# reczoo/RecBox

Hardware: AMD Instinct MI355X
Metric: samples/sec fwd+bwd, Criteo-shaped batch 65 536; embedding HBM GB/s vs roofline (higher is better)
Workload: dtype f32; 1 GPU; FM (recbox.ranking) Criteo-shaped 26 sparse + 13 dense, dim 16, batch 65536 per GPU, uniform ids (8 distinct batches resident in HBM, replayed in rotation), fused path, hipGraph replay (one captured step per resident batch), dense-grad autograd contract (persistent grad buffer, rows of the previous step re-zeroed), no optimiser step; global_batch=65536, batch_per_gpu=65536, parallelism=dp1

## Files before the change

### recbox_amd/csrc/rbx_bwd_common.h

```cpp
#pragma once
#include "rbx_internal.h"

namespace rbx {

constexpr int kSortThreads = 256;
#define RBX_SORT_ITEMS 8
constexpr int kSortItems = RBX_SORT_ITEMS;
constexpr int kSortTile = kSortThreads * kSortItems;
constexpr int kChainTiles = 64;
constexpr int kChainPasses = 4;
constexpr int kRadix = 256;
#define RBX_MAX_RADIX_BITS 8
constexpr int kMaxRadixBits = RBX_MAX_RADIX_BITS;
#define RBX_CHUNK 40
constexpr int kChunk = RBX_CHUNK;
constexpr unsigned kLocalBits = 26;
constexpr unsigned kLocalMask = (1u << kLocalBits) - 1u;
constexpr int kNumSamples = 256;

struct KeyField {
  const void* ids;
  long long stride_b;
  int stride_l;
  int vocab;
  int mask_id;
  int pad_id;
  unsigned row_base;
  unsigned lk_off;
  short seq_len;
  unsigned char dtype, pool;
  int reserved;
};
struct KeyPack { KeyField f[RBX_MAX_FIELDS]; };
// ... 2 lines not shown
  float* grad;
  float* grad2;
  const float* table;
  unsigned row_base;
  int out_off;
  short dim;
  short seq_len;
  unsigned char pool, slot;
  short reserved;
  int table_stride;
  int reserved2;
};
struct RedPack { RedField f[RBX_MAX_FIELDS]; };

struct SegPack {
  unsigned tile0[RBX_MAX_FIELDS + 1];
  unsigned lk0[RBX_MAX_FIELDS + 1];
  unsigned row0[RBX_MAX_FIELDS];
  unsigned char first_pass[RBX_MAX_FIELDS];
  int n;
};
static_assert(sizeof(KeyPack) + sizeof(SegPack) + 96 <= 4096, "build_keys_kernel's arguments must fit the 4 KiB kernarg segment");

__device__ __forceinline__ void seg_of_tile(const SegPack& S, unsigned tile, int* seg, unsigned* first, unsigned* count) {
  int lo = 0, hi = S.n - 1;
  while (lo < hi) {
    const int mid = (lo + hi + 1) >> 1;
    if (S.tile0[mid] <= tile) lo = mid; else hi = mid - 1;
  }
  *seg = lo;
  const unsigned f = S.lk0[lo] + (tile - S.tile0[lo]) * static_cast<unsigned>(kSortTile);
  const unsigned end = S.lk0[lo + 1];
  *first = f;
  *count = (end - f < static_cast<unsigned>(kSortTile)) ? end - f : static_cast<unsigned>(kSortTile);
}

template <int RB>
__device__ __forceinline__ unsigned seg_digit(unsigned key, unsigned sentinel, unsigned row0, int shift) {
  const unsigned local = (key == sentinel) ? 0xFFFFFFFFu : key - row0;
  return (local >> shift) & ((1u << RB) - 1u);
}

struct NumField {
  const void* ids;
  float* grad;
  long long stride_b;
  int out_off;
  short dim;
  unsigned char dtype, reserved;
};
struct NumPack { NumField f[RBX_MAX_FIELDS]; };

struct BwdPlan {
  int n_cat = 0, n_num = 0;
  KeyPack keys;
  RedPack red;
  NumPack num;
// ... 144 lines not shown
```

### recbox_amd/csrc/rbx_embed_bwd.hip

```cpp
#include <stdlib.h>
#include "rbx_segreduce.h"

namespace rbx {

static size_t align_up(size_t v, size_t a) { return (v + a - 1) / a * a; }

static int g_sort_chained = -1;
static bool sort_chained_on() {
  if (g_sort_chained < 0) {
    const char* e = getenv("RBX_SORT_CHAINED");
    g_sort_chained = (e != nullptr && e[0] == '0') ? 0 : 1;
  }
  return g_sort_chained != 0;
}

int make_plan(const rbx_field_t* fields, int n, int64_t B, const float* dout, int64_t stride_b, BwdPlan* p,
              int extra_dim, const unsigned long long* lookups_of) {
  if (fields == nullptr || n <= 0 || n > RBX_MAX_FIELDS) return fail(RBX_ERR_INVALID, "bad field array");
  FieldPack tmp;
  int rc = pack_fields(fields, n, B, true, &tmp);
  if (rc != RBX_OK) return rc;
  unsigned long long lookups = 0, rows = 0;
  const float* seen_table[RBX_MAX_FIELDS];
  unsigned seen_base[RBX_MAX_FIELDS];
// ... 79 lines not shown
    unsigned tiles = 0, lk = 0;
    unsigned long long max_rows = 1;
    unsigned long long rows_of_seg[RBX_MAX_FIELDS];
    int c = 0;
    while (c < p->n_cat) {
      int end = last_field_of_table[field_table[c]];
      unsigned long long seg_rows = 0;
      unsigned seg_lk = 0;
      const unsigned row0 = p->keys.f[c].row_base;
      int t_lo = field_table[c], t_hi = field_table[c];
      for (int k = c; k <= end; ++k) {
        if (last_field_of_table[field_table[k]] > end) end = last_field_of_table[field_table[k]];
        if (field_table[k] > t_hi) t_hi = field_table[k];
        if (field_table[k] < t_lo) t_lo = field_table[k];
        seg_lk += field_lookups[k];
      }
      for (int t = t_lo; t <= t_hi; ++t) seg_rows += static_cast<unsigned long long>(seen_vocab[t]);
      if (seg_lk > 0) {
        S.tile0[S.n] = tiles;
        S.lk0[S.n] = lk;
        S.row0[S.n] = row0;
        rows_of_seg[S.n] = seg_rows;
        ++S.n;
        tiles += (seg_lk + kSortTile - 1) / kSortTile;
        lk += seg_lk;
        if (seg_rows > max_rows) max_rows = seg_rows;
      }
      c = end + 1;
    }
    S.tile0[S.n] = tiles;
    S.lk0[S.n] = lk;
    p->n_tiles = tiles;
    unsigned max_nt = 0;
    for (int g = 0; g < S.n; ++g)
      if (S.tile0[g + 1] - S.tile0[g] > max_nt) max_nt = S.tile0[g + 1] - S.tile0[g];
    p->chained = max_nt <= static_cast<unsigned>(kChainTiles);
    int bits = 1;
    while ((1ull << bits) <= max_rows) ++bits;
    p->passes = (bits + kMaxRadixBits - 1) / kMaxRadixBits;
    const int per = (bits + p->passes - 1) / p->passes;
    p->radix_bits = per <= 8 ? 8 : (per <= 10 ? 10 : 11);
    for (int g = 0; g < S.n; ++g) {
      int sb = 1;
      while ((1ull << sb) <= rows_of_seg[g]) ++sb;
      const int need = (sb + p->radix_bits - 1) / p->radix_bits;
      S.first_pass[g] = static_cast<unsigned char>(p->passes - need);
    }
  }
  {
    int c = static_cast<int>(p->n_lookups / 32768u) / 8 * 8;
    if (c < 16) c = 16;
    if (c > kChunk) c = kChunk;
    p->chunk = c;
  }
  p->n_chunks = (p->n_lookups + p->chunk - 1) / p->chunk;
  p->num_blocks = static_cast<unsigned>((B + kNumSamples - 1) / kNumSamples);
  size_t o = 0;
  const size_t nl = align_up(static_cast<size_t>(p->n_lookups) * 4, 256);
  p->off_keys[0] = o; o += nl;
  p->off_keys[1] = o; o += nl;
  p->off_vals[0] = o; o += nl;
  p->off_vals[1] = o; o += nl;
  const size_t radix = static_cast<size_t>(1) << p->radix_bits;
  p->chained = sort_chained_on() && p->chained && p->passes <= kChainPasses && p->radix_bits == 8;
  p->off_hist = o;
  o += p->chained ? align_up((2 * static_cast<size_t>(p->n_tiles) * radix + p->n_tiles + static_cast<size_t>(p->segs.n) * radix) *
                             p->passes * 4, 256)
                  : align_up(static_cast<size_t>(p->n_tiles) * radix * 4 + 4, 256);
  p->off_ssum = o; o += align_up((static_cast<size_t>(p->n_tiles) * radix / 4096 + 2) * 4, 256);
  p->sum_stride = p->max_dim + extra_dim;
  p->off_head = o; o += align_up(static_cast<size_t>(p->n_chunks) * p->sum_stride * 4, 256);
  p->off_tail = o; o += align_up(static_cast<size_t>(p->n_chunks) * p->sum_stride * 4, 256);
  p->off_flags = o; o += align_up(static_cast<size_t>(p->n_chunks) * 4, 256);
  p->off_fin = o; o += align_up((2 * static_cast<size_t>(p->n_chunks) + 3 + kLongSlots) * 4, 256);
  p->off_long = o; o += align_up(static_cast<size_t>(kLongSlots) * p->sum_stride * 4, 256);
  p->off_num = o; o += align_up(static_cast<size_t>(p->n_num) * p->num_blocks * p->max_dim * 4, 256);
  p->bytes = o + 256;
  return RBX_OK;
}


template <int RB>
__global__ __launch_bounds__(kSortThreads) void build_keys_kernel(const KeyPack P, const int n_cat, const SegPack S,
                                                         const unsigned sentinel, unsigned* __restrict__ keys0,
                                                         unsigned* __restrict__ vals0, unsigned* __restrict__ keys1,
                                                         unsigned* __restrict__ vals1, int* __restrict__ status,
                                                         unsigned* __restrict__ fin, unsigned* __restrict__ hist,
                                                         const int chain_passes, const unsigned n_tiles) {
  constexpr int R = 1 << RB;
  constexpr int kCP = (RB == 8) ? kChainPasses : 1;
  if (blockIdx.x == 0 && threadIdx.x == 0) {
    fin[0] = 0;
    fin[1] = 0;
    fin[2] = 0;
  }
  __shared__ KeyField sf[RBX_MAX_FIELDS];
  {
    const int words = n_cat * static_cast<int>(sizeof(KeyField) / 4);
    const int* src = reinterpret_cast<const int*>(&P);
    int* dst = reinterpret_cast<int*>(sf);
    for (int i = threadIdx.x; i < words; i += blockDim.x) dst[i] = src[i];
  }
  __shared__ unsigned cnt[kCP][R];
  for (int d = threadIdx.x; d < kCP * R; d += kSortThreads) (&cnt[0][0])[d] = 0;
  __syncthreads();
  int seg;
  unsigned tile0, tile_n;
  seg_of_tile(S, blockIdx.x, &seg, &tile0, &tile_n);
  const unsigned row0 = S.row0[seg];
  const int fp = S.first_pass[seg];
  unsigned* __restrict__ keys = (fp & 1) ? keys1 : keys0;
  unsigned* __restrict__ vals = (fp & 1) ? vals1 : vals0;
#pragma unroll
  for (int it = 0; it < kSortItems; ++it) {
    const unsigned off = it * kSortThreads + threadIdx.x;
    if (off >= tile_n) break;
    const unsigned j = tile0 + off;
    int lo = 0, hi = n_cat - 1;
    while (lo < hi) {
      const int mid = (lo + hi + 1) >> 1;
      if (sf[mid].lk_off <= j) lo = mid; else hi = mid - 1;
    }
    const KeyField& fd = sf[lo];
    const unsigned local = j - fd.lk_off;
    const unsigned L = static_cast<unsigned>(fd.seq_len);
    const unsigned b = local / L;
    const unsigned l = local - b * L;
    const long long id = load_id(fd.ids, static_cast<long long>(b) * fd.stride_b + static_cast<long long>(l) * fd.stride_l,
                                 fd.dtype);
    unsigned key = sentinel;
    if (id < 0 || id >= fd.vocab) {
      if (status != nullptr) atomicOr(status, 1);
    } else {
      const bool id_pool = fd.pool == RBX_POOL_MEAN_ID || fd.pool == RBX_POOL_SUM_ID;
      if (id != fd.pad_id && !(id_pool && id == fd.mask_id)) key = fd.row_base + static_cast<unsigned>(id);
    }
    keys[j] = key;
    vals[j] = (static_cast<unsigned>(lo) << kLocalBits) | local;
    if (chain_passes > 0) {
#pragma unroll
      for (int k = 0; k < kCP; ++k)
        if (fp + k < chain_passes) atomicAdd(&cnt[k][seg_digit<RB>(key, sentinel, row0, k * RB)], 1u);
    } else if (fp == 0) {
      atomicAdd(&cnt[0][seg_digit<RB>(key, sentinel, row0, 0)], 1u);
    }
  }
  if (chain_passes > 0) {
    __syncthreads();
    const size_t plane = static_cast<size_t>(n_tiles) * R;
    unsigned* flags = hist + 2 * plane * chain_passes;
    for (int k = 0; fp + k < chain_passes; ++k) {
      unsigned* h = hist + plane * (fp + k) + static_cast<size_t>(blockIdx.x) * R;
      for (int d = threadIdx.x; d < R; d += kSortThreads) h[d] = cnt[k < kCP ? k : 0][d];
      if (threadIdx.x == 0) flags[static_cast<size_t>(fp + k) * n_tiles + blockIdx.x] = 0u;
    }
    return;
  }
  if (fp != 0) return;
  __syncthreads();
  const unsigned t_in = blockIdx.x - S.tile0[seg], nt = S.tile0[seg + 1] - S.tile0[seg];
  unsigned* h = hist + static_cast<size_t>(S.tile0[seg]) * R + t_in;
  for (int d = threadIdx.x; d < R; d += kSortThreads) h[static_cast<size_t>(d) * nt] = cnt[0][d];
}

template <int RB>
__global__ __launch_bounds__(kSortThreads) void radix_hist_kernel(const unsigned* __restrict__ keys, const SegPack S,
                                                                  const unsigned sentinel, const int pass,
                                                                  unsigned* __restrict__ hist) {
  constexpr int R = 1 << RB;
  __shared__ unsigned cnt[R];
  int seg;
  unsigned tile0, tile_n;
  seg_of_tile(S, blockIdx.x, &seg, &tile0, &tile_n);
  if (pass < S.first_pass[seg]) return;
  const int shift = (pass - S.first_pass[seg]) * RB;
  for (int d = threadIdx.x; d < R; d += kSortThreads) cnt[d] = 0;
  __syncthreads();
  const unsigned row0 = S.row0[seg];
#pragma unroll
  for (int i = 0; i < kSortItems; ++i) {
    const unsigned off = i * kSortThreads + threadIdx.x;
    if (off < tile_n) atomicAdd(&cnt[seg_digit<RB>(keys[tile0 + off], sentinel, row0, shift)], 1u);
  }
  __syncthreads();
  const unsigned t_in = blockIdx.x - S.tile0[seg], nt = S.tile0[seg + 1] - S.tile0[seg];
  unsigned* h = hist + static_cast<size_t>(S.tile0[seg]) * R + t_in;
  for (int d = threadIdx.x; d < R; d += kSortThreads) h[static_cast<size_t>(d) * nt] = cnt[d];
}

constexpr int kScanSlice = 4096;
constexpr int kMaxFusedSlices = 4 * kSortThreads;

__device__ __forceinline__ unsigned block_scan_1024x4(unsigned (&v)[4], unsigned* wave_tot, unsigned* total) {
  const int lane = threadIdx.x & 63, wid = threadIdx.x >> 6;
  const unsigned mine = v[0] + v[1] + v[2] + v[3];
  unsigned inc = mine;
#pragma unroll
  for (int o = 1; o < 64; o <<= 1) {
    const unsigned t = __shfl_up(inc, o, 64);
    if (lane >= o) inc += t;
  }
  if (lane == 63) wave_tot[wid] = inc;
  __syncthreads();
  unsigned wbase = 0, all = 0;
#pragma unroll
  for (int w = 0; w < 16; ++w) {
    const unsigned t = wave_tot[w];
    if (w < wid) wbase += t;
    all += t;
  }
  *total = all;
  return wbase + inc - mine;
}

// ... 14 lines not shown
  if (threadIdx.x == 0) slice_sum[blockIdx.x] = total;
}

__global__ __launch_bounds__(1024) void radix_scan_sums_kernel(unsigned* __restrict__ sums, const unsigned len) {
  __shared__ unsigned wave_tot[16];
  unsigned carry = 0;
  for (unsigned base = 0; base < len; base += kScanSlice) {
    const unsigned i0 = base + threadIdx.x * 4;
    unsigned v[4];
#pragma unroll
    for (int k = 0; k < 4; ++k) v[k] = (i0 + k < len) ? sums[i0 + k] : 0u;
    unsigned total;
    unsigned run = carry + block_scan_1024x4(v, wave_tot, &total);
#pragma unroll
    for (int k = 0; k < 4; ++k) {
      if (i0 + k < len) sums[i0 + k] = run;
      run += v[k];
    }
    carry += total;
    __syncthreads();
  }
}

template <int RB, bool CHAIN>
__global__ __launch_bounds__(kSortThreads) void radix_scatter_kernel(const unsigned* __restrict__ keys_in,
                                                                     const unsigned* __restrict__ vals_in,
                                                                     unsigned* __restrict__ keys_out,
                                                                     unsigned* __restrict__ vals_out, const SegPack S,
                                                                     const unsigned sentinel, const int pass,
                                                                     const unsigned* __restrict__ hist,
                                                                     const unsigned* __restrict__ slice_sum,
                                                                     const unsigned n_slices, const bool raw_sums,
                                                                     unsigned* __restrict__ chain, const int passes,
                                                                     const unsigned n_tiles) {
  constexpr int R = 1 << RB;
  constexpr int DPT = R / kSortThreads;
  constexpr int kWaves = kSortThreads / 64;
  constexpr int kPerWave = kSortTile / kWaves;
  constexpr int kSteps = kPerWave / 64;
  __shared__ unsigned wcnt[kWaves][R];
  __shared__ unsigned dstart[R];
  __shared__ unsigned gbase[R];
  __shared__ unsigned skey[kSortTile];
  __shared__ unsigned sval[kSortTile];
  const int lane = threadIdx.x & 63, wid = threadIdx.x >> 6;
  int seg;
  unsigned tile0, tile_n;
  seg_of_tile(S, blockIdx.x, &seg, &tile0, &tile_n);
  if (pass < S.first_pass[seg]) return;
  const int shift = (pass - S.first_pass[seg]) * RB;
  const unsigned row0 = S.row0[seg];
  const unsigned t_in = blockIdx.x - S.tile0[seg], nt = S.tile0[seg + 1] - S.tile0[seg];
  const size_t hfirst = static_cast<size_t>(S.tile0[seg]) * R;
  const size_t hbase = hfirst + t_in;
  const unsigned seg_lk0 = S.lk0[seg];
  for (int i = threadIdx.x; i < kWaves * R; i += kSortThreads) (&wcnt[0][0])[i] = 0;
  unsigned chain_excl[DPT], chain_before[DPT];
  const size_t plane = static_cast<size_t>(n_tiles) * R;
  const bool first_of_seg = pass == S.first_pass[seg];
  if constexpr (CHAIN) {
    __shared__ unsigned ctot[kWaves];
    const unsigned* T = chain + plane * pass + static_cast<size_t>(S.tile0[seg]) * R;
    unsigned* G = chain + (2 * plane + n_tiles) * passes;
    unsigned tot[DPT];
    unsigned mine = 0;
    if (first_of_seg) {
#pragma unroll
      for (int q = 0; q < DPT; ++q) {
        const int d = threadIdx.x * DPT + q;
        unsigned a = 0, b = 0;
#pragma unroll 8
        for (unsigned t = 0; t < nt; ++t) {
          const unsigned c = T[static_cast<size_t>(t) * R + d];
          a += c;
          b += (t < t_in) ? c : 0u;
        }
        tot[q] = a;
        chain_before[q] = b;
        mine += a;
      }
      if (t_in == 0) {
        for (int k = pass + 1; k < passes; ++k) {
          const unsigned* Tk = chain + plane * k + static_cast<size_t>(S.tile0[seg]) * R;
#pragma unroll
          for (int q = 0; q < DPT; ++q) {
            const int d = threadIdx.x * DPT + q;
            unsigned a = 0;
#pragma unroll 8
            for (unsigned t = 0; t < nt; ++t) a += Tk[static_cast<size_t>(t) * R + d];
            G[(static_cast<size_t>(k) * S.n + seg) * R + d] = a;
          }
        }
      }
    } else {
#pragma unroll
      for (int q = 0; q < DPT; ++q) {
        tot[q] = G[(static_cast<size_t>(pass) * S.n + seg) * R + threadIdx.x * DPT + q];
        chain_before[q] = 0;
        mine += tot[q];
      }
    }
    unsigned inc = mine;
#pragma unroll
    for (int o = 1; o < 64; o <<= 1) {
      const unsigned u = __shfl_up(inc, o, 64);
      if (lane >= o) inc += u;
    }
    if (lane == 63) ctot[wid] = inc;
    __syncthreads();
    unsigned run = inc - mine;
    for (int w = 0; w < wid; ++w) run += ctot[w];
#pragma unroll
    for (int q = 0; q < DPT; ++q) {
      chain_excl[q] = run;
      run += tot[q];
    }
  } else if (raw_sums) {
    __shared__ unsigned spre[kMaxFusedSlices];
    __shared__ unsigned stot[kWaves];
    const unsigned i0 = threadIdx.x * 4;
    unsigned t[4];
#pragma unroll
    for (int q = 0; q < 4; ++q) t[q] = (i0 + q < n_slices) ? slice_sum[i0 + q] : 0u;
    const unsigned mine = t[0] + t[1] + t[2] + t[3];
    unsigned inc = mine;
#pragma unroll
    for (int o = 1; o < 64; o <<= 1) {
      const unsigned u = __shfl_up(inc, o, 64);
      if (lane >= o) inc += u;
    }
    if (lane == 63) stot[wid] = inc;
    __syncthreads();
    unsigned run = inc - mine;
    for (int w = 0; w < wid; ++w) run += stot[w];
#pragma unroll
    for (int q = 0; q < 4; ++q) {
      spre[i0 + q] = run;
      run += t[q];
    }
    __syncthreads();
    const unsigned first = hist[hfirst] + spre[hfirst / kScanSlice];
    for (int d = threadIdx.x; d < R; d += kSortThreads) {
      const size_t hi = hbase + static_cast<size_t>(d) * nt;
      gbase[d] = seg_lk0 + (hist[hi] + spre[hi / kScanSlice] - first);
    }
  } else {
    const unsigned first = hist[hfirst] + slice_sum[hfirst / kScanSlice];
    for (int d = threadIdx.x; d < R; d += kSortThreads) {
      const size_t hi = hbase + static_cast<size_t>(d) * nt;
      gbase[d] = seg_lk0 + (hist[hi] + slice_sum[hi / kScanSlice] - first);
    }
  }
  __syncthreads();

  unsigned k[kSteps], v[kSteps];
  unsigned rank[kSteps];
  const unsigned long long lt = (lane == 0) ? 0ull : (~0ull >> (64 - lane));
#pragma unroll
  for (int s = 0; s < kSteps; ++s) {
    const unsigned off = wid * kPerWave + s * 64 + lane;
    const bool ok = off < tile_n;
    k[s] = ok ? __builtin_nontemporal_load(keys_in + tile0 + off) : 0xFFFFFFFFu;
    v[s] = ok ? __builtin_nontemporal_load(vals_in + tile0 + off) : 0u;
  }
#pragma unroll
  for (int s = 0; s < kSteps; ++s) {
    const unsigned off = wid * kPerWave + s * 64 + lane;
    const bool ok = off < tile_n;
    const unsigned d = ok ? seg_digit<RB>(k[s], sentinel, row0, shift) : 0u;
    unsigned long long peers = __ballot(ok);
#pragma unroll
    for (int b = 0; b < RB; ++b) {
      const unsigned long long m = __ballot((d >> b) & 1u);
      peers &= ((d >> b) & 1u) ? m : ~m;
    }
    if (!ok) peers = 0ull;
    const unsigned before = __popcll(peers & lt);
    volatile unsigned* wc = wcnt[wid];
    unsigned prev = 0;
    if (ok) prev = wc[d];
    rank[s] = prev + before;
    if (ok && before == 0) wc[d] = prev + __popcll(peers);
  }
  __syncthreads();
  {
    unsigned runs[DPT];
    unsigned mine = 0;
#pragma unroll
    for (int q = 0; q < DPT; ++q) {
      const int d = threadIdx.x * DPT + q;
      unsigned run = 0;
#pragma unroll
      for (int w = 0; w < kWaves; ++w) {
        const unsigned c = wcnt[w][d];
        wcnt[w][d] = run;
        run += c;
      }
      runs[q] = run;
      mine += run;
    }
    unsigned inc = mine;
#pragma unroll
    for (int o = 1; o < 64; o <<= 1) {
      const unsigned t = __shfl_up(inc, o, 64);
      if (lane >= o) inc += t;
    }
    __shared__ unsigned wtot[kWaves];
    if (lane == 63) wtot[wid] = inc;
    __syncthreads();
    unsigned base = inc - mine;
    for (int w = 0; w < wid; ++w) base += wtot[w];
#pragma unroll
    for (int q = 0; q < DPT; ++q) {
      dstart[threadIdx.x * DPT + q] = base;
      base += runs[q];
    }
    if constexpr (CHAIN) {
      if (!first_of_seg) {
        unsigned* L = chain + plane * (passes + pass);
        unsigned* flags = chain + 2 * plane * passes + static_cast<size_t>(pass) * n_tiles;
#pragma unroll
        for (int q = 0; q < DPT; ++q)
          __hip_atomic_store(L + static_cast<size_t>(blockIdx.x) * R + threadIdx.x * DPT + q, runs[q], __ATOMIC_RELAXED,
                             __HIP_MEMORY_SCOPE_AGENT);
        asm volatile("s_waitcnt vmcnt(0)" ::: "memory");
        __syncthreads();
        if (threadIdx.x == 0) __hip_atomic_store(flags + blockIdx.x, 1u, __ATOMIC_RELAXED, __HIP_MEMORY_SCOPE_AGENT);
        if (threadIdx.x < t_in) {
          const unsigned* f = flags + S.tile0[seg] + threadIdx.x;
          while (__hip_atomic_load(f, __ATOMIC_RELAXED, __HIP_MEMORY_SCOPE_AGENT) == 0u) __builtin_amdgcn_s_sleep(1);
        }
        __syncthreads();
        const unsigned* Ls = L + static_cast<size_t>(S.tile0[seg]) * R;
#pragma unroll
        for (int q = 0; q < DPT; ++q) {
          unsigned b = 0;
#pragma unroll 8
          for (unsigned t = 0; t < t_in; ++t)
            b += __hip_atomic_load(Ls + static_cast<size_t>(t) * R + threadIdx.x * DPT + q, __ATOMIC_RELAXED,
                                   __HIP_MEMORY_SCOPE_AGENT);
          chain_before[q] = b;
        }
      }
#pragma unroll
      for (int q = 0; q < DPT; ++q) gbase[threadIdx.x * DPT + q] = seg_lk0 + chain_excl[q] + chain_before[q];
    }
  }
  __syncthreads();
#pragma unroll
  for (int s = 0; s < kSteps; ++s) {
    const unsigned off = wid * kPerWave + s * 64 + lane;
    if (off < tile_n) {
      const unsigned d = seg_digit<RB>(k[s], sentinel, row0, shift);
      const unsigned pos = dstart[d] + wcnt[wid][d] + rank[s];
      skey[pos] = k[s];
      sval[pos] = v[s];
    }
  }
  __syncthreads();
#pragma unroll
  for (int i = 0; i < kSortItems; ++i) {
    const unsigned pos = i * kSortThreads + threadIdx.x;
    if (pos < tile_n) {
      const unsigned key = skey[pos];
      const unsigned d = seg_digit<RB>(key, sentinel, row0, shift);
      const unsigned g = gbase[d] + (pos - dstart[d]);
      keys_out[g] = key;
      vals_out[g] = sval[pos];
    }
  }
}

struct GenericPolicy {
  static constexpr bool kHasCount = false;
  struct Args {
    const float* dout;
    long long stride_b;
    const float* row_scale;
    long long B;
    int accumulate;
    const int* index;
  };
  template <class F>
  static __device__ __forceinline__ void contribute(const Args& a, const RedField& fd, unsigned local, int lane_g,
                                                    F& frag, float& cnt) {
// ... 95 lines not shown

}

extern "C" int rbx_sort_chained(int32_t enable) {
  const int was = rbx::sort_chained_on() ? 1 : 0;
  if (enable >= 0) rbx::g_sort_chained = enable ? 1 : 0;
  return was;
}

extern "C" size_t rbx_embed_bwd_workspace_size(const rbx_field_t* fields, int32_t n_fields, int64_t batch) {
  rbx::BwdPlan p;
  if (rbx::make_plan(fields, n_fields, batch, nullptr, 0, &p) != RBX_OK) return 0;
  return p.bytes;
}

namespace rbx {
template <int RB>
static int run_passes_rb(const BwdPlan& p, char* ws, hipStream_t s) {
  constexpr int R = 1 << RB;
  unsigned* keys[2] = {reinterpret_cast<unsigned*>(ws + p.off_keys[0]), reinterpret_cast<unsigned*>(ws + p.off_keys[1])};
  unsigned* vals[2] = {reinterpret_cast<unsigned*>(ws + p.off_vals[0]), reinterpret_cast<unsigned*>(ws + p.off_vals[1])};
  unsigned* hist = reinterpret_cast<unsigned*>(ws + p.off_hist);
  unsigned* ssum = reinterpret_cast<unsigned*>(ws + p.off_ssum);
  const bool chained = p.chained && RB == 8;
  int rc = RBX_OK;
  int cur = 0;
  for (int pass = 0; pass < p.passes; ++pass) {
    if (chained) {
      hipLaunchKernelGGL((radix_scatter_kernel<RB, true>), dim3(p.n_tiles), dim3(kSortThreads), 0, s, keys[cur], vals[cur],
                         keys[cur ^ 1], vals[cur ^ 1], p.segs, p.total_rows, pass, static_cast<const unsigned*>(nullptr),
                         static_cast<const unsigned*>(nullptr), 0u, false, hist, p.passes, p.n_tiles);
      rc = check_launch("radix pass (chained)");
      if (rc != RBX_OK) return rc;
      cur ^= 1;
      continue;
    }
    if (pass > 0)
      hipLaunchKernelGGL(radix_hist_kernel<RB>, dim3(p.n_tiles), dim3(kSortThreads), 0, s, keys[cur], p.segs, p.total_rows,
                         pass, hist);
    const unsigned hist_len = p.n_tiles * R;
    const unsigned n_slices = (hist_len + kScanSlice - 1) / kScanSlice;
    hipLaunchKernelGGL(radix_scan_local_kernel, dim3(n_slices), dim3(1024), 0, s, hist, hist_len, ssum);
    const bool raw_sums = n_slices <= static_cast<unsigned>(kMaxFusedSlices);
    if (!raw_sums) hipLaunchKernelGGL(radix_scan_sums_kernel, dim3(1), dim3(1024), 0, s, ssum, n_slices);
    hipLaunchKernelGGL((radix_scatter_kernel<RB, false>), dim3(p.n_tiles), dim3(kSortThreads), 0, s, keys[cur], vals[cur],
                       keys[cur ^ 1], vals[cur ^ 1], p.segs, p.total_rows, pass, hist, ssum, n_slices, raw_sums,
                       static_cast<unsigned*>(nullptr), p.passes, p.n_tiles);
    rc = check_launch("radix pass");
    if (rc != RBX_OK) return rc;
    cur ^= 1;
  }
  return RBX_OK;
}

int run_sort_passes(const BwdPlan& p, char* ws, hipStream_t s) {
  switch (p.radix_bits) {
    case 8: return run_passes_rb<8>(p, ws, s);
    case 10: return run_passes_rb<10>(p, ws, s);
    default: return run_passes_rb<11>(p, ws, s);
  }
}

template <int RB>
static int run_sort_rb(const BwdPlan& p, char* ws, int* d_status, hipStream_t s) {
  unsigned* keys[2] = {reinterpret_cast<unsigned*>(ws + p.off_keys[0]), reinterpret_cast<unsigned*>(ws + p.off_keys[1])};
  unsigned* vals[2] = {reinterpret_cast<unsigned*>(ws + p.off_vals[0]), reinterpret_cast<unsigned*>(ws + p.off_vals[1])};
  const bool chained = p.chained && RB == 8;
  hipLaunchKernelGGL(build_keys_kernel<RB>, dim3(p.n_tiles), dim3(kSortThreads), 0, s, p.keys, p.n_cat, p.segs, p.total_rows,
                     keys[0], vals[0], keys[1], vals[1], d_status, reinterpret_cast<unsigned*>(ws + p.off_fin),
                     reinterpret_cast<unsigned*>(ws + p.off_hist), chained ? p.passes : 0, p.n_tiles);
  const int rc = check_launch("build_keys_kernel");
  if (rc != RBX_OK) return rc;
  return run_passes_rb<RB>(p, ws, s);
}

int run_sort(const BwdPlan& p, char* ws, int* d_status, hipStream_t s) {
  if (p.n_lookups == 0) return RBX_OK;
  switch (p.radix_bits) {
    case 8: return run_sort_rb<8>(p, ws, d_status, s);
    case 10: return run_sort_rb<10>(p, ws, d_status, s);
    default: return run_sort_rb<11>(p, ws, d_status, s);
  }
}

int generic_reduce(const BwdPlan& p, const float* dout, int64_t stride_b, const int32_t* index, const float* row_scale,
                   int64_t B, int accumulate, char* ws, hipStream_t s) {
  for (int i = 0; i < p.n_cat; ++i) {
    const unsigned char pool = p.red.f[i].pool;
    if ((pool == RBX_POOL_MEAN_VALUE || pool == RBX_POOL_MEAN_ID) && row_scale == nullptr)
      return fail(RBX_ERR_INVALID, "mean pooling backward needs d_row_scale from the forward");
  }
// ... 72 lines not shown
```

### recbox_amd/csrc/rbx_embed_csr.hip

```cpp
#include "rbx_bwd_common.h"
#include "rbx_rowfrag.h"
#include "rbx_segreduce.h"

namespace rbx {

constexpr int kStatusBadId = 1;
constexpr int kStatusBadOffsets = 2;

struct BagK {
  const void* indices;
  const void* offsets;
  const float* table;
  long long idx_stride;
  int nnz;
  int vocab;
  int mask_id;
  int pad_id;
  int out_off;
  short dim;
  unsigned char idx_dtype, off_dtype, pool, slot;
  short reserved;
  float eps;
};
static_assert(sizeof(BagK) == 64, "BagK must stay 64 bytes");
// ... 573 lines not shown

static bool bag_vec_ok(const rbx_bag_t& g, const float* out, int64_t stride_b) {
  if (g.dim % 4 != 0 || g.out_off % 4 != 0 || stride_b % 4 != 0) return false;
  if ((reinterpret_cast<uintptr_t>(g.table) & 15) != 0) return false;
  if ((reinterpret_cast<uintptr_t>(out) & 15) != 0) return false;
  return true;
}

__global__ __launch_bounds__(256) void csr_bag_map_kernel(const BagPack P, const BagLookups LK, const long long B,
                                                          int* __restrict__ map, int* __restrict__ status) {
  const BagK& fd = P.f[blockIdx.y];
  int* __restrict__ my = map + LK.lk_off[blockIdx.y];
  const int lane = threadIdx.x & 15;
  for (long long b = static_cast<long long>(blockIdx.x) * 16 + (threadIdx.x >> 4); b < B;
       b += static_cast<long long>(gridDim.x) * 16) {
    int begin, end;
    bool bad;
    bag_range(fd, b, &begin, &end, &bad);
    if (bad && lane == 0 && status != nullptr) atomicOr(status, kStatusBadOffsets);
    for (int j = begin + lane; j < end; j += 16) my[j] = static_cast<int>(b);
  }
}

template <int RB, bool POS = false>
__global__ __launch_bounds__(kSortThreads) void csr_keys_kernel(const KeyPack P, const int n_cat, const SegPack S,
                                                                const unsigned sentinel, const int* __restrict__ map,
                                                                unsigned* __restrict__ keys0, unsigned* __restrict__ vals0,
                                                                unsigned* __restrict__ keys1, unsigned* __restrict__ vals1,
                                                                int* __restrict__ status, unsigned* __restrict__ fin,
                                                                unsigned* __restrict__ hist, const int chain_passes,
                                                                const unsigned n_tiles) {
  constexpr int R = 1 << RB;
  constexpr int kCP = (RB == 8) ? kChainPasses : 1;
  if (blockIdx.x == 0 && threadIdx.x == 0) {
    fin[0] = 0;
    fin[1] = 0;
    fin[2] = 0;
  }
  __shared__ KeyField sf[RBX_MAX_FIELDS];
  {
    const int words = n_cat * static_cast<int>(sizeof(KeyField) / 4);
    const int* src = reinterpret_cast<const int*>(&P);
    int* dst = reinterpret_cast<int*>(sf);
    for (int i = threadIdx.x; i < words; i += blockDim.x) dst[i] = src[i];
  }
  __shared__ unsigned cnt[kCP][R];
  for (int d = threadIdx.x; d < kCP * R; d += kSortThreads) (&cnt[0][0])[d] = 0;
  __syncthreads();
  int seg;
  unsigned tile0, tile_n;
  seg_of_tile(S, blockIdx.x, &seg, &tile0, &tile_n);
  const unsigned row0 = S.row0[seg];
  const int fp = S.first_pass[seg];
  unsigned* __restrict__ keys = (fp & 1) ? keys1 : keys0;
  unsigned* __restrict__ vals = (fp & 1) ? vals1 : vals0;
#pragma unroll
  for (int it = 0; it < kSortItems; ++it) {
    const unsigned off = it * kSortThreads + threadIdx.x;
    if (off >= tile_n) break;
    const unsigned j = tile0 + off;
    int lo = 0, hi = n_cat - 1;
    while (lo < hi) {
      const int mid = (lo + hi + 1) >> 1;
      if (sf[mid].lk_off <= j) lo = mid; else hi = mid - 1;
    }
    const KeyField& fd = sf[lo];
    const unsigned local = j - fd.lk_off;
    const int bag = map[j];
    unsigned key = sentinel;
    if (bag >= 0) {
      const long long id = load_id(fd.ids, static_cast<long long>(local) * fd.stride_b, fd.dtype);
      if (id < 0 || id >= fd.vocab) {
        if (status != nullptr) atomicOr(status, kStatusBadId);
      } else {
        const bool id_pool = fd.pool == RBX_POOL_MEAN_ID || fd.pool == RBX_POOL_SUM_ID;
        if (id != fd.pad_id && !(id_pool && id == fd.mask_id)) key = fd.row_base + static_cast<unsigned>(id);
      }
    }
    keys[j] = key;
    if constexpr (POS) vals[j] = (static_cast<unsigned>(lo) << kLocalBits) | local;
    else vals[j] = (static_cast<unsigned>(lo) << kLocalBits) | static_cast<unsigned>(bag < 0 ? 0 : bag);
    if (chain_passes > 0) {
#pragma unroll
      for (int k = 0; k < kCP; ++k)
        if (fp + k < chain_passes) atomicAdd(&cnt[k][seg_digit<RB>(key, sentinel, row0, k * RB)], 1u);
    } else if (fp == 0) {
      atomicAdd(&cnt[0][seg_digit<RB>(key, sentinel, row0, 0)], 1u);
    }
  }
  if (chain_passes > 0) {
    __syncthreads();
    const size_t plane = static_cast<size_t>(n_tiles) * R;
    unsigned* flags = hist + 2 * plane * chain_passes;
    for (int k = 0; fp + k < chain_passes; ++k) {
      unsigned* h = hist + plane * (fp + k) + static_cast<size_t>(blockIdx.x) * R;
      for (int d = threadIdx.x; d < R; d += kSortThreads) h[d] = cnt[k < kCP ? k : 0][d];
      if (threadIdx.x == 0) flags[static_cast<size_t>(fp + k) * n_tiles + blockIdx.x] = 0u;
    }
    return;
  }
  if (fp != 0) return;
  __syncthreads();
  const unsigned t_in = blockIdx.x - S.tile0[seg], nt = S.tile0[seg + 1] - S.tile0[seg];
  unsigned* h = hist + static_cast<size_t>(S.tile0[seg]) * R + t_in;
  for (int d = threadIdx.x; d < R; d += kSortThreads) h[static_cast<size_t>(d) * nt] = cnt[0][d];
}

struct CsrPlan {
  BwdPlan p;
  BagPack bags;
  BagLookups lk;
  size_t off_map = 0, bytes = 0;
};

static int csr_plan(const rbx_bag_t* bags, int n, int64_t batch, const float* dout, int64_t stride_b, CsrPlan* c) {
  BagK all[RBX_MAX_BAGS];
  int rc = pack_bags(bags, n, batch, all);
  if (rc != RBX_OK) return rc;
  rbx_field_t fields[RBX_MAX_BAGS];
  unsigned long long lookups_of[RBX_MAX_BAGS];
  for (int i = 0; i < n; ++i) {
    const rbx_bag_t& g = bags[i];
    rbx_field_t& f = fields[i];
    f.ids = g.indices != nullptr ? g.indices : static_cast<const void*>(g.table);
    f.table = g.table;
    f.grad = g.grad;
    f.ids_stride_b = g.indices_stride;
    f.ids_stride_l = 0;
// ... 17 lines not shown
    if (bags[i].grad == nullptr) continue;
    c->bags.f[k] = all[i];
    c->lk.lk_off[k] = c->p.keys.f[k].lk_off;
    ++k;
  }
  c->off_map = c->p.bytes;
  c->bytes = c->p.bytes + (static_cast<size_t>(c->p.n_lookups) * 4 + 255) / 256 * 256;
  return RBX_OK;
}

int csr_bwd_plan(const rbx_bag_t* bags, int n, int64_t batch, BwdPlan* p, size_t* bytes) {
  CsrPlan c;
  const int rc = csr_plan(bags, n, batch, nullptr, 0, &c);
  if (rc != RBX_OK) return rc;
  *p = c.p;
  *bytes = c.bytes;
  return RBX_OK;
}

template <int RB, bool POS = false>
static int launch_csr_keys(const CsrPlan& c, char* ws, int* status, hipStream_t s) {
  const BwdPlan& p = c.p;
  const bool chained = p.chained && RB == 8;
  hipLaunchKernelGGL((csr_keys_kernel<RB, POS>), dim3(p.n_tiles), dim3(kSortThreads), 0, s, p.keys, p.n_cat, p.segs, p.total_rows,
                     reinterpret_cast<const int*>(ws + c.off_map), reinterpret_cast<unsigned*>(ws + p.off_keys[0]),
                     reinterpret_cast<unsigned*>(ws + p.off_vals[0]), reinterpret_cast<unsigned*>(ws + p.off_keys[1]),
                     reinterpret_cast<unsigned*>(ws + p.off_vals[1]), status, reinterpret_cast<unsigned*>(ws + p.off_fin),
                     reinterpret_cast<unsigned*>(ws + p.off_hist), chained ? p.passes : 0, p.n_tiles);
  return check_launch("csr_keys_kernel");
}

struct BagPolicyBase {
  static constexpr bool kHasCount = false;
  template <class A>
  static __device__ __forceinline__ float weight(const A&, float w) { return w; }
  template <class A, class F>
  static __device__ __forceinline__ void prefetch(const A& a, const RedField& fd, unsigned row, int lane_g, F& pre) {
    if (a.accumulate) pre.add_from(fd.grad + static_cast<size_t>(row) * fd.dim, fd.dim, lane_g);
  }
  template <class A, class F>
  static __device__ __forceinline__ void prefetch_raw(const A& a, const RedField& fd, unsigned row, int lane_g, F& pre) {
    if (a.accumulate) pre.load_from(fd.grad + static_cast<size_t>(row) * fd.dim, fd.dim, lane_g);
  }
  template <class A, class F>
  static __device__ __forceinline__ void flush(const A&, const RedField& fd, unsigned row, const F& acc, float, const F& pre,
                                               int lane_g) {
    F out = acc;
// ... 581 lines not shown
```

Baseline: 327.6 million samples/s.

## Template radix sort on tile geometry and parallelize chained histogram walk across waves

Parameterizes the sort kernels by a SortGeom struct covering threads and items per tile, so the tile size becomes a compile-time choice. The chain limit is now expressed as a pair count rather than a tile count. The chained scatter's first-of-segment walk over per-tile digit counts is split across waves, each summing a range of tiles with coalesced lane-indexed reads, then combined through shared memory. Before, each thread serially walked all tiles for its own digits. This adds two extra barriers and reuses skey/sval as scratch, and guards digit-owner threads for geometries where threads exceed the radix.

```diff
diff --git a/recbox_amd/csrc/rbx_bwd_common.h b/recbox_amd/csrc/rbx_bwd_common.h
--- a/recbox_amd/csrc/rbx_bwd_common.h
+++ b/recbox_amd/csrc/rbx_bwd_common.h
@@ -3,12 +3,30 @@
 
 namespace rbx {
 
-constexpr int kSortThreads = 256;
+constexpr int kChainPairs = 64 * 2048;
+constexpr int kChainPasses = 4;
+template <int THREADS, int ITEMS>
+struct SortGeom {
+  static constexpr int kThreads = THREADS;
+  static constexpr int kItems = ITEMS;
+  static constexpr int kTile = THREADS * ITEMS;
+  static constexpr int kWaves = THREADS / 64;
+  static constexpr int kPerWave = kTile / kWaves;
+  static constexpr int kSteps = kPerWave / 64;
+  static constexpr int kChainTiles = kChainPairs / kTile;
+  static constexpr int kMaxFusedSlices = 4 * THREADS;
+  static_assert(THREADS % 64 == 0 && THREADS >= 64 && THREADS <= 1024, "whole wavefronts, one workgroup");
+  static_assert(kWaves * kPerWave == kTile && kSteps * 64 == kPerWave && kSteps == ITEMS, "tile order is (wave, step, lane)");
+  static_assert(kChainTiles * kTile == kChainPairs, "the chained sort's limit is a whole number of tiles");
+  static_assert(kChainTiles <= THREADS, "radix_scatter_kernel<RB, true>: one thread per earlier tile of the segment reads its flag");
+};
+#ifndef RBX_SORT_THREADS
+#define RBX_SORT_THREADS 256
+#endif
+#ifndef RBX_SORT_ITEMS
 #define RBX_SORT_ITEMS 8
-constexpr int kSortItems = RBX_SORT_ITEMS;
-constexpr int kSortTile = kSortThreads * kSortItems;
-constexpr int kChainTiles = 64;
-constexpr int kChainPasses = 4;
+#endif
+using SortGeo = SortGeom<RBX_SORT_THREADS, RBX_SORT_ITEMS>;
 constexpr int kRadix = 256;
 #define RBX_MAX_RADIX_BITS 8
 constexpr int kMaxRadixBits = RBX_MAX_RADIX_BITS;
@@ -57,6 +75,7 @@
 };
 static_assert(sizeof(KeyPack) + sizeof(SegPack) + 96 <= 4096, "build_keys_kernel's arguments must fit the 4 KiB kernarg segment");
 
+template <int TILE>
 __device__ __forceinline__ void seg_of_tile(const SegPack& S, unsigned tile, int* seg, unsigned* first, unsigned* count) {
   int lo = 0, hi = S.n - 1;
   while (lo < hi) {
@@ -64,10 +83,10 @@
     if (S.tile0[mid] <= tile) lo = mid; else hi = mid - 1;
   }
   *seg = lo;
-  const unsigned f = S.lk0[lo] + (tile - S.tile0[lo]) * static_cast<unsigned>(kSortTile);
+  const unsigned f = S.lk0[lo] + (tile - S.tile0[lo]) * static_cast<unsigned>(TILE);
   const unsigned end = S.lk0[lo + 1];
   *first = f;
-  *count = (end - f < static_cast<unsigned>(kSortTile)) ? end - f : static_cast<unsigned>(kSortTile);
+  *count = (end - f < static_cast<unsigned>(TILE)) ? end - f : static_cast<unsigned>(TILE);
 }
 
 template <int RB>
diff --git a/recbox_amd/csrc/rbx_embed_bwd.hip b/recbox_amd/csrc/rbx_embed_bwd.hip
--- a/recbox_amd/csrc/rbx_embed_bwd.hip
+++ b/recbox_amd/csrc/rbx_embed_bwd.hip
@@ -125,7 +125,7 @@
         S.row0[S.n] = row0;
         rows_of_seg[S.n] = seg_rows;
         ++S.n;
-        tiles += (seg_lk + kSortTile - 1) / kSortTile;
+        tiles += (seg_lk + SortGeo::kTile - 1) / SortGeo::kTile;
         lk += seg_lk;
         if (seg_rows > max_rows) max_rows = seg_rows;
       }
@@ -137,7 +137,7 @@
     unsigned max_nt = 0;
     for (int g = 0; g < S.n; ++g)
       if (S.tile0[g + 1] - S.tile0[g] > max_nt) max_nt = S.tile0[g + 1] - S.tile0[g];
-    p->chained = max_nt <= static_cast<unsigned>(kChainTiles);
+    p->chained = max_nt <= static_cast<unsigned>(SortGeo::kChainTiles);
     int bits = 1;
     while ((1ull << bits) <= max_rows) ++bits;
     p->passes = (bits + kMaxRadixBits - 1) / kMaxRadixBits;
@@ -183,8 +183,8 @@
 }
 
 
-template <int RB>
-__global__ __launch_bounds__(kSortThreads) void build_keys_kernel(const KeyPack P, const int n_cat, const SegPack S,
+template <int RB, class G>
+__global__ __launch_bounds__(G::kThreads) void build_keys_kernel(const KeyPack P, const int n_cat, const SegPack S,
                                                          const unsigned sentinel, unsigned* __restrict__ keys0,
                                                          unsigned* __restrict__ vals0, unsigned* __restrict__ keys1,
                                                          unsigned* __restrict__ vals1, int* __restrict__ status,
@@ -205,18 +205,18 @@
     for (int i = threadIdx.x; i < words; i += blockDim.x) dst[i] = src[i];
   }
   __shared__ unsigned cnt[kCP][R];
-  for (int d = threadIdx.x; d < kCP * R; d += kSortThreads) (&cnt[0][0])[d] = 0;
+  for (int d = threadIdx.x; d < kCP * R; d += G::kThreads) (&cnt[0][0])[d] = 0;
   __syncthreads();
   int seg;
   unsigned tile0, tile_n;
-  seg_of_tile(S, blockIdx.x, &seg, &tile0, &tile_n);
+  seg_of_tile<G::kTile>(S, blockIdx.x, &seg, &tile0, &tile_n);
   const unsigned row0 = S.row0[seg];
   const int fp = S.first_pass[seg];
   unsigned* __restrict__ keys = (fp & 1) ? keys1 : keys0;
   unsigned* __restrict__ vals = (fp & 1) ? vals1 : vals0;
 #pragma unroll
-  for (int it = 0; it < kSortItems; ++it) {
-    const unsigned off = it * kSortThreads + threadIdx.x;
+  for (int it = 0; it < G::kItems; ++it) {
+    const unsigned off = it * G::kThreads + threadIdx.x;
     if (off >= tile_n) break;
     const unsigned j = tile0 + off;
     int lo = 0, hi = n_cat - 1;
@@ -254,7 +254,7 @@
     unsigned* flags = hist + 2 * plane * chain_passes;
     for (int k = 0; fp + k < chain_passes; ++k) {
       unsigned* h = hist + plane * (fp + k) + static_cast<size_t>(blockIdx.x) * R;
-      for (int d = threadIdx.x; d < R; d += kSortThreads) h[d] = cnt[k < kCP ? k : 0][d];
+      for (int d = threadIdx.x; d < R; d += G::kThreads) h[d] = cnt[k < kCP ? k : 0][d];
       if (threadIdx.x == 0) flags[static_cast<size_t>(fp + k) * n_tiles + blockIdx.x] = 0u;
     }
     return;
@@ -263,36 +263,35 @@
   __syncthreads();
   const unsigned t_in = blockIdx.x - S.tile0[seg], nt = S.tile0[seg + 1] - S.tile0[seg];
   unsigned* h = hist + static_cast<size_t>(S.tile0[seg]) * R + t_in;
-  for (int d = threadIdx.x; d < R; d += kSortThreads) h[static_cast<size_t>(d) * nt] = cnt[0][d];
-}
-
-template <int RB>
-__global__ __launch_bounds__(kSortThreads) void radix_hist_kernel(const unsigned* __restrict__ keys, const SegPack S,
+  for (int d = threadIdx.x; d < R; d += G::kThreads) h[static_cast<size_t>(d) * nt] = cnt[0][d];
+}
+
+template <int RB, class G>
+__global__ __launch_bounds__(G::kThreads) void radix_hist_kernel(const unsigned* __restrict__ keys, const SegPack S,
                                                                   const unsigned sentinel, const int pass,
                                                                   unsigned* __restrict__ hist) {
   constexpr int R = 1 << RB;
   __shared__ unsigned cnt[R];
   int seg;
   unsigned tile0, tile_n;
-  seg_of_tile(S, blockIdx.x, &seg, &tile0, &tile_n);
+  seg_of_tile<G::kTile>(S, blockIdx.x, &seg, &tile0, &tile_n);
   if (pass < S.first_pass[seg]) return;
   const int shift = (pass - S.first_pass[seg]) * RB;
-  for (int d = threadIdx.x; d < R; d += kSortThreads) cnt[d] = 0;
+  for (int d = threadIdx.x; d < R; d += G::kThreads) cnt[d] = 0;
   __syncthreads();
   const unsigned row0 = S.row0[seg];
 #pragma unroll
-  for (int i = 0; i < kSortItems; ++i) {
-    const unsigned off = i * kSortThreads + threadIdx.x;
+  for (int i = 0; i < G::kItems; ++i) {
+    const unsigned off = i * G::kThreads + threadIdx.x;
     if (off < tile_n) atomicAdd(&cnt[seg_digit<RB>(keys[tile0 + off], sentinel, row0, shift)], 1u);
   }
   __syncthreads();
   const unsigned t_in = blockIdx.x - S.tile0[seg], nt = S.tile0[seg + 1] - S.tile0[seg];
   unsigned* h = hist + static_cast<size_t>(S.tile0[seg]) * R + t_in;
-  for (int d = threadIdx.x; d < R; d += kSortThreads) h[static_cast<size_t>(d) * nt] = cnt[d];
+  for (int d = threadIdx.x; d < R; d += G::kThreads) h[static_cast<size_t>(d) * nt] = cnt[d];
 }
 
 constexpr int kScanSlice = 4096;
-constexpr int kMaxFusedSlices = 4 * kSortThreads;
 
 __device__ __forceinline__ unsigned block_scan_1024x4(unsigned (&v)[4], unsigned* wave_tot, unsigned* total) {
   const int lane = threadIdx.x & 63, wid = threadIdx.x >> 6;
@@ -353,8 +352,8 @@
   }
 }
 
-template <int RB, bool CHAIN>
-__global__ __launch_bounds__(kSortThreads) void radix_scatter_kernel(const unsigned* __restrict__ keys_in,
+template <int RB, bool CHAIN, class G>
+__global__ __launch_bounds__(G::kThreads) void radix_scatter_kernel(const unsigned* __restrict__ keys_in,
                                                                      const unsigned* __restrict__ vals_in,
                                                                      unsigned* __restrict__ keys_out,
                                                                      unsigned* __restrict__ vals_out, const SegPack S,
@@ -365,19 +364,25 @@
                                                                      unsigned* __restrict__ chain, const int passes,
                                                                      const unsigned n_tiles) {
   constexpr int R = 1 << RB;
-  constexpr int DPT = R / kSortThreads;
-  constexpr int kWaves = kSortThreads / 64;
-  constexpr int kPerWave = kSortTile / kWaves;
-  constexpr int kSteps = kPerWave / 64;
+  constexpr int DPT = R > G::kThreads ? R / G::kThreads : 1;
+  constexpr int kDigThreads = R / DPT;
+  static_assert(kDigThreads * DPT == R && kDigThreads <= G::kThreads, "every digit has one owner thread");
+  constexpr int kWaves = G::kWaves;
+  constexpr int kPerWave = G::kPerWave;
+  constexpr int kSteps = G::kSteps;
+  constexpr int kMaxFusedSlices = G::kMaxFusedSlices;
+  static_assert(kMaxFusedSlices == 4 * G::kThreads, "raw_sums: a thread scans four slice totals");
+  static_assert(!CHAIN || kWaves * R <= G::kTile, "the chained walk keeps a row of partial counts per wave in skey / sval");
   __shared__ unsigned wcnt[kWaves][R];
   __shared__ unsigned dstart[R];
   __shared__ unsigned gbase[R];
-  __shared__ unsigned skey[kSortTile];
-  __shared__ unsigned sval[kSortTile];
+  __shared__ unsigned skey[G::kTile];
+  __shared__ unsigned sval[G::kTile];
   const int lane = threadIdx.x & 63, wid = threadIdx.x >> 6;
+  const bool dig = kDigThreads == G::kThreads || threadIdx.x < kDigThreads;
   int seg;
   unsigned tile0, tile_n;
-  seg_of_tile(S, blockIdx.x, &seg, &tile0, &tile_n);
+  seg_of_tile<G::kTile>(S, blockIdx.x, &seg, &tile0, &tile_n);
   if (pass < S.first_pass[seg]) return;
   const int shift = (pass - S.first_pass[seg]) * RB;
   const unsigned row0 = S.row0[seg];
@@ -385,49 +390,75 @@
   const size_t hfirst = static_cast<size_t>(S.tile0[seg]) * R;
   const size_t hbase = hfirst + t_in;
   const unsigned seg_lk0 = S.lk0[seg];
-  for (int i = threadIdx.x; i < kWaves * R; i += kSortThreads) (&wcnt[0][0])[i] = 0;
+  for (int i = threadIdx.x; i < kWaves * R; i += G::kThreads) (&wcnt[0][0])[i] = 0;
   unsigned chain_excl[DPT], chain_before[DPT];
   const size_t plane = static_cast<size_t>(n_tiles) * R;
   const bool first_of_seg = pass == S.first_pass[seg];
   if constexpr (CHAIN) {
     __shared__ unsigned ctot[kWaves];
     const unsigned* T = chain + plane * pass + static_cast<size_t>(S.tile0[seg]) * R;
-    unsigned* G = chain + (2 * plane + n_tiles) * passes;
+    unsigned* G_ = chain + (2 * plane + n_tiles) * passes;
     unsigned tot[DPT];
     unsigned mine = 0;
+#pragma unroll
+    for (int q = 0; q < DPT; ++q) tot[q] = chain_before[q] = 0;
     if (first_of_seg) {
-#pragma unroll
-      for (int q = 0; q < DPT; ++q) {
-        const int d = threadIdx.x * DPT + q;
-        unsigned a = 0, b = 0;
-#pragma unroll 8
-        for (unsigned t = 0; t < nt; ++t) {
-          const unsigned c = T[static_cast<size_t>(t) * R + d];
-          a += c;
-          b += (t < t_in) ? c : 0u;
+      constexpr int DPL = R / 64;
+      const unsigned per = (nt + kWaves - 1) / kWaves;
+      const unsigned t_lo = wid * per;
+      const unsigned t_hi = (t_lo + per < nt) ? t_lo + per : nt;
+      auto walk = [&](const unsigned* __restrict__ Tk, const unsigned before_tile, unsigned (&all)[DPT], unsigned (&before)[DPT]) {
+        unsigned a[DPL], b[DPL];
+#pragma unroll
+        for (int j = 0; j < DPL; ++j) a[j] = b[j] = 0;
+#pragma unroll 4
+        for (unsigned t = t_lo; t < t_hi; ++t) {
+#pragma unroll
+          for (int j = 0; j < DPL; ++j) {
+            const unsigned c = Tk[static_cast<size_t>(t) * R + j * 64 + lane];
+            a[j] += c;
+            b[j] += (t < before_tile) ? c : 0u;
+          }
         }
-        tot[q] = a;
-        chain_before[q] = b;
-        mine += a;
-      }
+#pragma unroll
+        for (int j = 0; j < DPL; ++j) {
+          skey[wid * R + j * 64 + lane] = a[j];
+          sval[wid * R + j * 64 + lane] = b[j];
+        }
+        __syncthreads();
+        if (dig) {
+#pragma unroll
+          for (int q = 0; q < DPT; ++q) {
+            const int d = threadIdx.x * DPT + q;
+            unsigned sa = 0, sb = 0;
+#pragma unroll
+            for (int w = 0; w < kWaves; ++w) {
+              sa += skey[w * R + d];
+              sb += sval[w * R + d];
+            }
+            all[q] = sa;
+            before[q] = sb;
+          }
+        }
+        __syncthreads();
+      };
+      walk(T, t_in, tot, chain_before);
+#pragma unroll
+      for (int q = 0; q < DPT; ++q) mine += tot[q];
       if (t_in == 0) {
         for (int k = pass + 1; k < passes; ++k) {
-          const unsigned* Tk = chain + plane * k + static_cast<size_t>(S.tile0[seg]) * R;
-#pragma unroll
-          for (int q = 0; q < DPT; ++q) {
-            const int d = threadIdx.x * DPT + q;
-            unsigned a = 0;
-#pragma unroll 8
-            for (unsigned t = 0; t < nt; ++t) a += Tk[static_cast<size_t>(t) * R + d];
-            G[(static_cast<size_t>(k) * S.n + seg) * R + d] = a;
+          unsigned gt[DPT], none[DPT];
+          walk(chain + plane * k + static_cast<size_t>(S.tile0[seg]) * R, 0u, gt, none);
+          if (dig) {
+#pragma unroll
+            for (int q = 0; q < DPT; ++q) G_[(static_cast<size_t>(k) * S.n + seg) * R + threadIdx.x * DPT + q] = gt[q];
           }
         }
       }
-    } else {
+    } else if (dig) {
 #pragma unroll
       for (int q = 0; q < DPT; ++q) {
-        tot[q] = G[(static_cast<size_t>(pass) * S.n + seg) * R + threadIdx.x * DPT + q];
-        chain_before[q] = 0;
+        tot[q] = G_[(static_cast<size_t>(pass) * S.n + seg) * R + threadIdx.x * DPT + q];
         mine += tot[q];
       }
     }
@@ -471,13 +502,13 @@
     }
     __syncthreads();
     const unsigned first = hist[hfirst] + spre[hfirst / kScanSlice];
-    for (int d = threadIdx.x; d < R; d += kSortThreads) {
+    for (int d = threadIdx.x; d < R; d += G::kThreads) {
       const size_t hi = hbase + static_cast<size_t>(d) * nt;
       gbase[d] = seg_lk0 + (hist[hi] + spre[hi / kScanSlice] - first);
     }
   } else {
     const unsigned first = hist[hfirst] + slice_sum[hfirst / kScanSlice];
-    for (int d = threadIdx.x; d < R; d += kSortThreads) {
+    for (int d = threadIdx.x; d < R; d += G::kThreads) {
       const size_t hi = hbase + static_cast<size_t>(d) * nt;
       gbase[d] = seg_lk0 + (hist[hi] + slice_sum[hi / kScanSlice] - first);
     }
@@ -521,11 +552,13 @@
     for (int q = 0; q < DPT; ++q) {
       const int d = threadIdx.x * DPT + q;
       unsigned run = 0;
-#pragma unroll
-      for (int w = 0; w < kWaves; ++w) {
-        const unsigned c = wcnt[w][d];
-        wcnt[w][d] = run;
-        run += c;
+      if (dig) {
+#pragma unroll
+        for (int w = 0; w < kWaves; ++w) {
+          const unsigned c = wcnt[w][d];
+          wcnt[w][d] = run;
+          run += c;
+        }
       }
       runs[q] = run;
       mine += run;
@@ -543,7 +576,7 @@
     for (int w = 0; w < wid; ++w) base += wtot[w];
 #pragma unroll
     for (int q = 0; q < DPT; ++q) {
-      dstart[threadIdx.x * DPT + q] = base;
+      if (dig) dstart[threadIdx.x * DPT + q] = base;
       base += runs[q];
     }
     if constexpr (CHAIN) {
@@ -552,8 +585,9 @@
         unsigned* flags = chain + 2 * plane * passes + static_cast<size_t>(pass) * n_tiles;
 #pragma unroll
         for (int q = 0; q < DPT; ++q)
-          __hip_atomic_store(L + static_cast<size_t>(blockIdx.x) * R + threadIdx.x * DPT + q, runs[q], __ATOMIC_RELAXED,
-                             __HIP_MEMORY_SCOPE_AGENT);
+          if (dig)
+            __hip_atomic_store(L + static_cast<size_t>(blockIdx.x) * R + threadIdx.x * DPT + q, runs[q], __ATOMIC_RELAXED,
+                               __HIP_MEMORY_SCOPE_AGENT);
         asm volatile("s_waitcnt vmcnt(0)" ::: "memory");
         __syncthreads();
         if (threadIdx.x == 0) __hip_atomic_store(flags + blockIdx.x, 1u, __ATOMIC_RELAXED, __HIP_MEMORY_SCOPE_AGENT);
@@ -567,14 +601,15 @@
         for (int q = 0; q < DPT; ++q) {
           unsigned b = 0;
 #pragma unroll 8
-          for (unsigned t = 0; t < t_in; ++t)
+          for (unsigned t = 0; t < (dig ? t_in : 0u); ++t)
             b += __hip_atomic_load(Ls + static_cast<size_t>(t) * R + threadIdx.x * DPT + q, __ATOMIC_RELAXED,
                                    __HIP_MEMORY_SCOPE_AGENT);
           chain_before[q] = b;
         }
       }
 #pragma unroll
-      for (int q = 0; q < DPT; ++q) gbase[threadIdx.x * DPT + q] = seg_lk0 + chain_excl[q] + chain_before[q];
+      for (int q = 0; q < DPT; ++q)
+        if (dig) gbase[threadIdx.x * DPT + q] = seg_lk0 + chain_excl[q] + chain_before[q];
     }
   }
   __syncthreads();
@@ -590,8 +625,8 @@
   }
   __syncthreads();
 #pragma unroll
-  for (int i = 0; i < kSortItems; ++i) {
-    const unsigned pos = i * kSortThreads + threadIdx.x;
+  for (int i = 0; i < G::kItems; ++i) {
+    const unsigned pos = i * G::kThreads + threadIdx.x;
     if (pos < tile_n) {
       const unsigned key = skey[pos];
       const unsigned d = seg_digit<RB>(key, sentinel, row0, shift);
@@ -733,12 +768,11 @@
   unsigned* vals[2] = {reinterpret_cast<unsigned*>(ws + p.off_vals[0]), reinterpret_cast<unsigned*>(ws + p.off_vals[1])};
   unsigned* hist = reinterpret_cast<unsigned*>(ws + p.off_hist);
   unsigned* ssum = reinterpret_cast<unsigned*>(ws + p.off_ssum);
-  const bool chained = p.chained && RB == 8;
   int rc = RBX_OK;
   int cur = 0;
   for (int pass = 0; pass < p.passes; ++pass) {
-    if (chained) {
-      hipLaunchKernelGGL((radix_scatter_kernel<RB, true>), dim3(p.n_tiles), dim3(kSortThreads), 0, s, keys[cur], vals[cur],
+    if constexpr (RB == 8) if (p.chained) {
+      hipLaunchKernelGGL((radix_scatter_kernel<RB, true, SortGeo>), dim3(p.n_tiles), dim3(SortGeo::kThreads), 0, s, keys[cur], vals[cur],
                          keys[cur ^ 1], vals[cur ^ 1], p.segs, p.total_rows, pass, static_cast<const unsigned*>(nullptr),
                          static_cast<const unsigned*>(nullptr), 0u, false, hist, p.passes, p.n_tiles);
       rc = check_launch("radix pass (chained)");
@@ -747,14 +781,14 @@
       continue;
     }
     if (pass > 0)
-      hipLaunchKernelGGL(radix_hist_kernel<RB>, dim3(p.n_tiles), dim3(kSortThreads), 0, s, keys[cur], p.segs, p.total_rows,
+      hipLaunchKernelGGL((radix_hist_kernel<RB, SortGeo>), dim3(p.n_tiles), dim3(SortGeo::kThreads), 0, s, keys[cur], p.segs, p.total_rows,
                          pass, hist);
     const unsigned hist_len = p.n_tiles * R;
     const unsigned n_slices = (hist_len + kScanSlice - 1) / kScanSlice;
     hipLaunchKernelGGL(radix_scan_local_kernel, dim3(n_slices), dim3(1024), 0, s, hist, hist_len, ssum);
-    const bool raw_sums = n_slices <= static_cast<unsigned>(kMaxFusedSlices);
+    const bool raw_sums = n_slices <= static_cast<unsigned>(SortGeo::kMaxFusedSlices);
     if (!raw_sums) hipLaunchKernelGGL(radix_scan_sums_kernel, dim3(1), dim3(1024), 0, s, ssum, n_slices);
-    hipLaunchKernelGGL((radix_scatter_kernel<RB, false>), dim3(p.n_tiles), dim3(kSortThreads), 0, s, keys[cur], vals[cur],
+    hipLaunchKernelGGL((radix_scatter_kernel<RB, false, SortGeo>), dim3(p.n_tiles), dim3(SortGeo::kThreads), 0, s, keys[cur], vals[cur],
                        keys[cur ^ 1], vals[cur ^ 1], p.segs, p.total_rows, pass, hist, ssum, n_slices, raw_sums,
                        static_cast<unsigned*>(nullptr), p.passes, p.n_tiles);
     rc = check_launch("radix pass");
@@ -777,7 +811,7 @@
   unsigned* keys[2] = {reinterpret_cast<unsigned*>(ws + p.off_keys[0]), reinterpret_cast<unsigned*>(ws + p.off_keys[1])};
   unsigned* vals[2] = {reinterpret_cast<unsigned*>(ws + p.off_vals[0]), reinterpret_cast<unsigned*>(ws + p.off_vals[1])};
   const bool chained = p.chained && RB == 8;
-  hipLaunchKernelGGL(build_keys_kernel<RB>, dim3(p.n_tiles), dim3(kSortThreads), 0, s, p.keys, p.n_cat, p.segs, p.total_rows,
+  hipLaunchKernelGGL((build_keys_kernel<RB, SortGeo>), dim3(p.n_tiles), dim3(SortGeo::kThreads), 0, s, p.keys, p.n_cat, p.segs, p.total_rows,
                      keys[0], vals[0], keys[1], vals[1], d_status, reinterpret_cast<unsigned*>(ws + p.off_fin),
                      reinterpret_cast<unsigned*>(ws + p.off_hist), chained ? p.passes : 0, p.n_tiles);
   const int rc = check_launch("build_keys_kernel");
diff --git a/recbox_amd/csrc/rbx_embed_csr.hip b/recbox_amd/csrc/rbx_embed_csr.hip
--- a/recbox_amd/csrc/rbx_embed_csr.hip
+++ b/recbox_amd/csrc/rbx_embed_csr.hip
@@ -619,8 +619,8 @@
   }
 }
 
-template <int RB, bool POS = false>
-__global__ __launch_bounds__(kSortThreads) void csr_keys_kernel(const KeyPack P, const int n_cat, const SegPack S,
+template <int RB, class G, bool POS = false>
+__global__ __launch_bounds__(G::kThreads) void csr_keys_kernel(const KeyPack P, const int n_cat, const SegPack S,
                                                                 const unsigned sentinel, const int* __restrict__ map,
                                                                 unsigned* __restrict__ keys0, unsigned* __restrict__ vals0,
                                                                 unsigned* __restrict__ keys1, unsigned* __restrict__ vals1,
@@ -642,18 +642,18 @@
     for (int i = threadIdx.x; i < words; i += blockDim.x) dst[i] = src[i];
   }
   __shared__ unsigned cnt[kCP][R];
-  for (int d = threadIdx.x; d < kCP * R; d += kSortThreads) (&cnt[0][0])[d] = 0;
+  for (int d = threadIdx.x; d < kCP * R; d += G::kThreads) (&cnt[0][0])[d] = 0;
   __syncthreads();
   int seg;
   unsigned tile0, tile_n;
-  seg_of_tile(S, blockIdx.x, &seg, &tile0, &tile_n);
+  seg_of_tile<G::kTile>(S, blockIdx.x, &seg, &tile0, &tile_n);
   const unsigned row0 = S.row0[seg];
   const int fp = S.first_pass[seg];
   unsigned* __restrict__ keys = (fp & 1) ? keys1 : keys0;
   unsigned* __restrict__ vals = (fp & 1) ? vals1 : vals0;
 #pragma unroll
-  for (int it = 0; it < kSortItems; ++it) {
-    const unsigned off = it * kSortThreads + threadIdx.x;
+  for (int it = 0; it < G::kItems; ++it) {
+    const unsigned off = it * G::kThreads + threadIdx.x;
     if (off >= tile_n) break;
     const unsigned j = tile0 + off;
     int lo = 0, hi = n_cat - 1;
@@ -691,7 +691,7 @@
     unsigned* flags = hist + 2 * plane * chain_passes;
     for (int k = 0; fp + k < chain_passes; ++k) {
       unsigned* h = hist + plane * (fp + k) + static_cast<size_t>(blockIdx.x) * R;
-      for (int d = threadIdx.x; d < R; d += kSortThreads) h[d] = cnt[k < kCP ? k : 0][d];
+      for (int d = threadIdx.x; d < R; d += G::kThreads) h[d] = cnt[k < kCP ? k : 0][d];
       if (threadIdx.x == 0) flags[static_cast<size_t>(fp + k) * n_tiles + blockIdx.x] = 0u;
     }
     return;
@@ -700,7 +700,7 @@
   __syncthreads();
   const unsigned t_in = blockIdx.x - S.tile0[seg], nt = S.tile0[seg + 1] - S.tile0[seg];
   unsigned* h = hist + static_cast<size_t>(S.tile0[seg]) * R + t_in;
-  for (int d = threadIdx.x; d < R; d += kSortThreads) h[static_cast<size_t>(d) * nt] = cnt[0][d];
+  for (int d = threadIdx.x; d < R; d += G::kThreads) h[static_cast<size_t>(d) * nt] = cnt[0][d];
 }
 
 struct CsrPlan {
@@ -764,7 +764,7 @@
 static int launch_csr_keys(const CsrPlan& c, char* ws, int* status, hipStream_t s) {
   const BwdPlan& p = c.p;
   const bool chained = p.chained && RB == 8;
-  hipLaunchKernelGGL((csr_keys_kernel<RB, POS>), dim3(p.n_tiles), dim3(kSortThreads), 0, s, p.keys, p.n_cat, p.segs, p.total_rows,
+  hipLaunchKernelGGL((csr_keys_kernel<RB, SortGeo, POS>), dim3(p.n_tiles), dim3(SortGeo::kThreads), 0, s, p.keys, p.n_cat, p.segs, p.total_rows,
                      reinterpret_cast<const int*>(ws + c.off_map), reinterpret_cast<unsigned*>(ws + p.off_keys[0]),
                      reinterpret_cast<unsigned*>(ws + p.off_vals[0]), reinterpret_cast<unsigned*>(ws + p.off_keys[1]),
                      reinterpret_cast<unsigned*>(ws + p.off_vals[1]), status, reinterpret_cast<unsigned*>(ws + p.off_fin),
```

Result: no change. 329.6 million samples/s, median of 3 (+0.6%).
